# DecaYale/RNNPose

Measured on AMD Instinct MI355X. Metric: pose-refine iters/sec (640x480, B=8, 3x8 recurrent), higher is better.
Workload: dtype f32 (convolutions and volume build: fp16x3-split MFMA, fp32-class accuracy; LM: f64)

## Files before the change

rnnpose_amd/csrc/lm.hip:

```cpp
#include "geometry.cuh"

namespace {

using rp::Intr;
using rp::Pose;

constexpr int NACC = 27;
constexpr int PSTRIDE = 32;
constexpr int LM_THREADS = 256;
#ifndef RP_LM_BATCH
#define RP_LM_BATCH 8
#endif
#ifndef RP_LM_PPB
#define RP_LM_PPB 4096
#endif
constexpr int LM_BATCH = RP_LM_BATCH;
constexpr int LM_PIX_PER_BLOCK = RP_LM_PPB;
constexpr int LM_MAX_BLOCKS = 256;

__host__ __device__ inline int lm_blocks_per_image(long long P) {
  long long n = (P + LM_PIX_PER_BLOCK - 1) / LM_PIX_PER_BLOCK;
  if (n < 1) n = 1;
  if (n > LM_MAX_BLOCKS) n = LM_MAX_BLOCKS;
  return static_cast<int>(n);
}

__device__ __forceinline__ double shfl_down_f64(double v, int d) {
  int lo = __double2loint(v), hi = __double2hiint(v);
  lo = __shfl_down(lo, d);
  hi = __shfl_down(hi, d);
  return __hiloint2double(hi, lo);
}

struct LmTail {
  int* tickets;
  double* Hm;
  double* bv;
  const float* G_in;
  float* G_out;
  float* xi;
  int* info;
  double ep, lm, max_update;
};
__device__ void lm_finalize_block_one(const double* __restrict__ partials, int nblk, int b, double* __restrict__ Hm, double* __restrict__ bv);
__device__ __forceinline__ void lm_solve_one(const double* Hm, const double* bv, const float* G, int b, double ep, double lm, double max_update,
                             float* G_new, float* xi_out, int* info);

__device__ __forceinline__ void lm_accumulate(double (&acc)[NACC], float wgt, float dep, float tx, float ty, int x, int y, int target_mode,
                                          float eps, const Intr& k, const Pose& g) {
  const float Z = dep + eps;
  if (target_mode != 0) {
    tx += static_cast<float>(x);
    ty += static_cast<float>(y);
  }
  const rp::Reproj r = rp::reproject(Z, static_cast<float>(x), static_cast<float>(y), k, g);
  const bool valid = (r.Z0 > rp::kMinDepthValid) && (r.Z1 > rp::kMinDepthValid);
  const double vw = valid ? static_cast<double>(wgt) : 0.0;
  const bool tiny = r.Zc <= rp::kMinDepthProj + 0.01f;
  const float zi1 = tiny ? 0.f : 1.0f / r.Zc;
  const float zi2 = tiny ? 0.f : 1.0f / (r.Zc * r.Zc);
  const double a = static_cast<double>(k.fx * zi1);
  const double c = static_cast<double>(-k.fx * r.X1 * zi2);
  const double d = static_cast<double>(k.fy * zi1);
  const double e = static_cast<double>(-k.fy * r.Y1 * zi2);
  const double X1 = r.X1, Y1 = r.Y1, Z1 = r.Z1;
  double J0[6], J1[6];
  J0[0] = a;   J0[1] = 0.0; J0[2] = c; J0[3] = c * Y1;            J0[4] = a * Z1 + c * (-X1); J0[5] = a * (-Y1);
  J1[0] = 0.0; J1[1] = d;   J1[2] = e; J1[3] = d * (-Z1) + e * Y1; J1[4] = e * (-X1);          J1[5] = d * X1;
  const double r0 = static_cast<double>(tx) - static_cast<double>(r.u);
  const double r1 = static_cast<double>(ty) - static_cast<double>(r.v);
  int idx = 0;
#pragma unroll
  for (int i = 0; i < 6; ++i) {
    const double wi0 = vw * J0[i], wi1 = vw * J1[i];
#pragma unroll
    for (int jj = i; jj < 6; ++jj) {
      acc[idx] += wi0 * J0[jj] + wi1 * J1[jj];
      ++idx;
    }
    acc[21 + i] += wi0 * r0 + wi1 * r1;
  }
}

template <bool FUSED>
__device__ __forceinline__ void lm_reduce_tail(double (&acc)[NACC], double* __restrict__ partials, const LmTail& tail, int b, int nblk, int bx) {
  __shared__ double red[LM_THREADS / 64][NACC];
  __shared__ int is_last;
  const int lane = threadIdx.x & 63, wave = threadIdx.x >> 6;
  {
    double v[32];
#pragma unroll
    for (int i = 0; i < 32; ++i) v[i] = i < NACC ? acc[i] : 0.0;
#pragma unroll
    for (int o = 32, n = 32; o >= 2; o >>= 1, n >>= 1) {
      const bool hi = (lane & o) != 0;
#pragma unroll
      for (int i = 0; i < n / 2; ++i) {
        const double send = hi ? v[i] : v[i + n / 2];
        const double keep = hi ? v[i + n / 2] : v[i];
        v[i] = keep + rp::shfl_xor_f64(send, o);
      }
    }
    const double tot = v[0] + rp::shfl_xor_f64(v[0], 1);
    const int slot = ((lane >> 5) & 1) * 16 + ((lane >> 4) & 1) * 8 + ((lane >> 3) & 1) * 4 + ((lane >> 2) & 1) * 2 + ((lane >> 1) & 1);
    if (!(lane & 1) && slot < NACC) red[wave][slot] = tot;
  }
  __syncthreads();
  if (threadIdx.x < NACC) {
    double v = red[0][threadIdx.x];
#pragma unroll
    for (int wv = 1; wv < LM_THREADS / 64; ++wv) v += red[wv][threadIdx.x];
    partials[(static_cast<long long>(b) * nblk + bx) * PSTRIDE + threadIdx.x] = v;
  }
  if constexpr (FUSED) {
    asm volatile("s_waitcnt vmcnt(0)" ::: "memory");
    __syncthreads();
    if (threadIdx.x == 0) {
      __builtin_amdgcn_fence(__ATOMIC_RELEASE, "agent");
      asm volatile("s_waitcnt vmcnt(0)" ::: "memory");
      const int t = __hip_atomic_fetch_add(&tail.tickets[b], 1, __ATOMIC_RELAXED, __HIP_MEMORY_SCOPE_AGENT);
      is_last = (t == nblk - 1) ? 1 : 0;
      if (is_last) {
        __hip_atomic_store(&tail.tickets[b], 0, __ATOMIC_RELAXED, __HIP_MEMORY_SCOPE_AGENT);
        __builtin_amdgcn_fence(__ATOMIC_ACQUIRE, "agent");
      }
    }
    __syncthreads();
    if (!is_last) return;
    lm_finalize_block_one(partials, nblk, b, tail.Hm, tail.bv);
    __syncthreads();
    if (threadIdx.x == 0) lm_solve_one(tail.Hm, tail.bv, tail.G_in, b, tail.ep, tail.lm, tail.max_update, tail.G_out, tail.xi, tail.info);
  }
}

template <bool FUSED>
__global__ __launch_bounds__(LM_THREADS) void lm_normal_eq_kernel(const float* __restrict__ target, int target_mode,
                                                                  const float* __restrict__ weight,
                                                                  const float* __restrict__ depth, float eps,
                                                                  const float* __restrict__ K,
                                                                  const float* __restrict__ G, int H, int W,
                                                                  double* __restrict__ partials, const LmTail tail) {
  const int b = blockIdx.y;
  const int nblk = gridDim.x;
  const long long P = static_cast<long long>(H) * W;
  const Intr k = rp::load_intr(K, b);
  const Pose g = rp::load_pose(G, b);
  double acc[NACC];
#pragma unroll
  for (int i = 0; i < NACC; ++i) acc[i] = 0.0;

  const long long stride = static_cast<long long>(nblk) * LM_THREADS;
  for (long long t0 = static_cast<long long>(blockIdx.x) * LM_THREADS + threadIdx.x; t0 < P; t0 += LM_BATCH * stride) {
    float wgt_[LM_BATCH], dep_[LM_BATCH], tx_[LM_BATCH], ty_[LM_BATCH];
#pragma unroll
    for (int j = 0; j < LM_BATCH; ++j) {
      const long long tj = t0 + j * stride;
      const long long t = tj < P ? tj : P - 1;
      wgt_[j] = weight[b * P + t];
      dep_[j] = depth[b * P + t];
      if (target_mode == 0) {
        const float2 tt = *reinterpret_cast<const float2*>(target + (b * P + t) * 2);
        tx_[j] = tt.x;
        ty_[j] = tt.y;
      } else {
        tx_[j] = target[(static_cast<long long>(b) * 2 + 0) * P + t];
        ty_[j] = target[(static_cast<long long>(b) * 2 + 1) * P + t];
      }
    }
    __builtin_amdgcn_sched_barrier(0);
#pragma unroll
    for (int j = 0; j < LM_BATCH; ++j) {
      const long long t = t0 + j * stride;
      if (t >= P) break;
      const unsigned tu = static_cast<unsigned>(t);
      const int y = static_cast<int>(tu / static_cast<unsigned>(W)), x = static_cast<int>(tu - static_cast<unsigned>(y) * static_cast<unsigned>(W));
      const float wgt = wgt_[j];
      const bool skippable = wgt == 0.f && __builtin_isfinite(tx_[j]) && __builtin_isfinite(ty_[j]) && __builtin_isfinite(dep_[j]);
      if (__builtin_amdgcn_ballot_w64(!skippable) == 0ull) continue;
      lm_accumulate(acc, wgt, dep_[j], tx_[j], ty_[j], x, y, target_mode, eps, k, g);
    }
  }
  lm_reduce_tail<FUSED>(acc, partials, tail, b, nblk, static_cast<int>(blockIdx.x));
}

__device__ void lm_finalize_block_one(const double* __restrict__ partials, int nblk, int b, double* __restrict__ Hm,
                                      double* __restrict__ bv) {
  __shared__ double grp[8][PSTRIDE];
  __shared__ double s[NACC];
  const int k = threadIdx.x & 31, g = threadIdx.x >> 5;
  double v = 0.0;
  for (int i = g; i < nblk; i += 8) v += partials[(static_cast<long long>(b) * nblk + i) * PSTRIDE + k];
  grp[g][k] = v;
  __syncthreads();
  if (threadIdx.x < NACC) {
    double t = 0.0;
    for (int q = 0; q < 8; ++q) t += grp[q][threadIdx.x];
    s[threadIdx.x] = t;
  }
  __syncthreads();
  if (threadIdx.x < 36) {
    const int i = threadIdx.x / 6, j = threadIdx.x % 6;
    const int r = i < j ? i : j, c = i < j ? j : i;
    const int idx = r * 6 - r * (r - 1) / 2 + (c - r);
    Hm[b * 36 + threadIdx.x] = s[idx];
  } else if (threadIdx.x < 42) {
    bv[b * 6 + (threadIdx.x - 36)] = s[21 + (threadIdx.x - 36)];
  }
}

__global__ __launch_bounds__(256) void lm_finalize_kernel(const double* __restrict__ partials, int nblk,
                                                          double* __restrict__ Hm, double* __restrict__ bv) {
  lm_finalize_block_one(partials, nblk, blockIdx.x, Hm, bv);
}

__device__ void se3_exp_dev(const float* xi, float* Gout ) {
  const float v0 = xi[0], v1 = xi[1], v2 = xi[2];
  const float w0 = xi[3], w1 = xi[4], w2 = xi[5];
  const float th2 = w0 * w0 + w1 * w1 + w2 * w2;
  const float th = sqrtf(th2);
  const float th4 = th2 * th2;
  const float wx[9] = {0.f, -w2, w1, w2, 0.f, -w0, -w1, w0, 0.f};
  float wx2[9];
  for (int i = 0; i < 3; ++i)
    for (int j = 0; j < 3; ++j) wx2[i * 3 + j] = wx[i * 3 + 0] * wx[0 * 3 + j] + wx[i * 3 + 1] * wx[1 * 3 + j] + wx[i * 3 + 2] * wx[2 * 3 + j];
  float A, Bc, Cc;
  float Bv;
  const float eps = 1e-12f;
  if (th < rp::kMinTheta) {
    A = 1.0f - (1.0f / 6.0f) * th2 + (1.0f / 120.0f) * th4;
    Bc = 0.5f - (1.0f / 12.0f) * th2 + (1.0f / 720.0f) * th4;
    Bv = 0.5f - (1.0f / 24.0f) * th2 + (1.0f / 720.0f) * th4;
    Cc = (1.0f / 6.0f) - (1.0f / 120.0f) * th2 + (1.0f / 5040.0f) * th4;
  } else {
    A = sinf(th) / (th + eps);
    Bc = (1.0f - cosf(th)) / (th2 + eps);
    Bv = Bc;
    Cc = (th - sinf(th)) / (th2 * th + eps);
  }
  float Rm[9], Vm[9];
  for (int i = 0; i < 9; ++i) {
    const float I = (i == 0 || i == 4 || i == 8) ? 1.f : 0.f;
    Rm[i] = I + A * wx[i] + Bc * wx2[i];
    Vm[i] = I + Bv * wx[i] + Cc * wx2[i];
  }
  for (int i = 0; i < 3; ++i) {
    Gout[i * 4 + 0] = Rm[i * 3 + 0];
    Gout[i * 4 + 1] = Rm[i * 3 + 1];
    Gout[i * 4 + 2] = Rm[i * 3 + 2];
    Gout[i * 4 + 3] = Vm[i * 3 + 0] * v0 + Vm[i * 3 + 1] * v1 + Vm[i * 3 + 2] * v2;
  }
  Gout[12] = 0.f; Gout[13] = 0.f; Gout[14] = 0.f; Gout[15] = 1.f;
}

__device__ void mat4_mul(const float* A, const float* Bm, float* C) {
  for (int i = 0; i < 4; ++i)
    for (int j = 0; j < 4; ++j) {
      float s = 0.f;
      for (int k = 0; k < 4; ++k) s += A[i * 4 + k] * Bm[k * 4 + j];
      C[i * 4 + j] = s;
    }
}

__device__ __forceinline__ void lm_solve_one(const double* Hm, const double* bv, const float* G, int b, double ep, double lm,
                                             double max_update, float* G_new , float* xi_out, int* info) {
  double L[21], xv[6];
#define LT(i_, j_) L[(i_) * ((i_) + 1) / 2 + (j_)]
#pragma unroll
  for (int i = 0; i < 6; ++i) {
#pragma unroll
    for (int j = 0; j <= i; ++j) LT(i, j) = Hm[b * 36 + i * 6 + j];
    xv[i] = bv[b * 6 + i];
  }
#pragma unroll
  for (int i = 0; i < 6; ++i) LT(i, i) = LT(i, i) + ep + lm * LT(i, i);
  int bad = 0;
  const double nan = __longlong_as_double(0x7ff8000000000000LL);
#pragma unroll
  for (int j = 0; j < 6; ++j) {
    double s = LT(j, j);
#pragma unroll
    for (int k = 0; k < j; ++k) s -= LT(j, k) * LT(j, k);
    if (!(s > 0.0)) {
      if (!bad) bad = j + 1;
      LT(j, j) = nan;
    } else {
      LT(j, j) = sqrt(s);
    }
#pragma unroll
    for (int i = j + 1; i < 6; ++i) {
      double t = LT(i, j);
#pragma unroll
      for (int k = 0; k < j; ++k) t -= LT(i, k) * LT(j, k);
      LT(i, j) = t / LT(j, j);
    }
  }
#pragma unroll
  for (int i = 0; i < 6; ++i) {
    double t = xv[i];
#pragma unroll
    for (int k = 0; k < i; ++k) t -= LT(i, k) * xv[k];
    xv[i] = t / LT(i, i);
  }
#pragma unroll
  for (int i = 5; i >= 0; --i) {
    double t = xv[i];
#pragma unroll
    for (int k = i + 1; k < 6; ++k) t -= LT(k, i) * xv[k];
    xv[i] = t / LT(i, i);
  }
#undef LT
  float xi[6];
  for (int i = 0; i < 6; ++i) {
    double v = xv[i];
    if (v != v) v = 0.0;
    v = v < -max_update ? -max_update : (v > max_update ? max_update : v);
    xi[i] = static_cast<float>(v);
    xi_out[b * 6 + i] = xi[i];
  }
  if (info) info[b] = bad;
  float dG[16], Gin[16], Gout[16];
  se3_exp_dev(xi, dG);
  for (int i = 0; i < 16; ++i) Gin[i] = G[b * 16 + i];
  mat4_mul(dG, Gin, Gout);
  for (int i = 0; i < 16; ++i) G_new[b * 16 + i] = Gout[i];
}

__global__ __launch_bounds__(64) void lm_solve_update_kernel(const double* __restrict__ Hm, const double* __restrict__ bv,
                                                             const float* G, int B, double ep, double lm,
                                                             double max_update, float* G_new ,
                                                             float* __restrict__ xi_out, int* __restrict__ info) {
  const int b = blockIdx.x * blockDim.x + threadIdx.x;
  if (b < B) lm_solve_one(Hm, bv, G, b, ep, lm, max_update, G_new, xi_out, info);
}

__global__ void se3_exp_kernel(const float* __restrict__ xi, int B, float* __restrict__ out) {
  const int b = blockIdx.x * blockDim.x + threadIdx.x;
  if (b >= B) return;
  float x[6], Gm[16];
  for (int i = 0; i < 6; ++i) x[i] = xi[b * 6 + i];
  se3_exp_dev(x, Gm);
  for (int i = 0; i < 16; ++i) out[b * 16 + i] = Gm[i];
}

__global__ void se3_compose_kernel(const float* __restrict__ A, const float* __restrict__ Bm, int B, float* __restrict__ out) {
  const int b = blockIdx.x * blockDim.x + threadIdx.x;
  if (b >= B) return;
  float a[16], c[16], o[16];
  for (int i = 0; i < 16; ++i) {
    a[i] = A[b * 16 + i];
    c[i] = Bm[b * 16 + i];
  }
  mat4_mul(a, c, o);
  for (int i = 0; i < 16; ++i) out[b * 16 + i] = o[i];
}

__global__ void se3_inverse_kernel(const float* __restrict__ A, int B, float* __restrict__ out) {
  const int b = blockIdx.x * blockDim.x + threadIdx.x;
  if (b >= B) return;
  float a[16], o[16];
  for (int i = 0; i < 16; ++i) a[i] = A[b * 16 + i];
  for (int i = 0; i < 3; ++i) {
    for (int j = 0; j < 3; ++j) o[i * 4 + j] = a[j * 4 + i];
    float s = 0.f;
    for (int k = 0; k < 3; ++k) s += a[k * 4 + i] * a[k * 4 + 3];
    o[i * 4 + 3] = -s;
  }
  o[12] = 0.f; o[13] = 0.f; o[14] = 0.f; o[15] = 1.f;
  for (int i = 0; i < 16; ++i) out[b * 16 + i] = o[i];
}

__global__ void se3_outer_update_kernel(const float* __restrict__ Tij, const float* __restrict__ Ti, int B, int literal, float* __restrict__ Ti_out,
                                        float* __restrict__ Tij_out) {
  const int b = blockIdx.x * blockDim.x + threadIdx.x;
  if (b >= B) return;
  float a[16], c[16], t[16], inv[16], o[16];
  for (int i = 0; i < 16; ++i) {
    a[i] = Tij[b * 16 + i];
    c[i] = Ti[b * 16 + i];
  }
  mat4_mul(a, c, t);
  for (int i = 0; i < 16; ++i) Ti_out[b * 16 + i] = t[i];
  if (literal) {
    for (int i = 0; i < 3; ++i) {
      for (int j = 0; j < 3; ++j) inv[i * 4 + j] = t[j * 4 + i];
      float s = 0.f;
      for (int k = 0; k < 3; ++k) s += t[k * 4 + i] * t[k * 4 + 3];
      inv[i * 4 + 3] = -s;
    }
    inv[12] = 0.f; inv[13] = 0.f; inv[14] = 0.f; inv[15] = 1.f;
    mat4_mul(t, inv, o);
  } else {
    for (int i = 0; i < 16; ++i) o[i] = (i % 5 == 0) ? 1.f : 0.f;
  }
  for (int i = 0; i < 16; ++i) Tij_out[b * 16 + i] = o[i];
}

inline double* lm_partials(void* workspace, int B) { return static_cast<double*>(workspace) + B; }

int launch_normal_eq_partials(const float* target, int target_mode, const float* weight, const float* depth, float eps,
                              const float* K, const float* G, int B, int H, int W, void* workspace, hipStream_t st) {
  const long long P = static_cast<long long>(H) * W;
  const int nblk = lm_blocks_per_image(P);
  hipLaunchKernelGGL(lm_normal_eq_kernel<false>, dim3(nblk, B), dim3(LM_THREADS), 0, st, target, target_mode, weight, depth, eps,
                     K, G, H, W, lm_partials(workspace, B), LmTail{});
  return nblk;
}

void launch_lm_step_fused(const float* target, int target_mode, const float* weight, const float* depth, float eps, const float* K,
                          const float* G_in, float* G_out, int B, int H, int W, double ep, double lm, double max_update,
                          void* workspace, double* Hm, double* bv, float* xi, int* info, hipStream_t st) {
  const long long P = static_cast<long long>(H) * W;
  const int nblk = lm_blocks_per_image(P);
  LmTail tail{};
  tail.tickets = static_cast<int*>(workspace);
  tail.Hm = Hm; tail.bv = bv; tail.G_in = G_in; tail.G_out = G_out; tail.xi = xi; tail.info = info;
  tail.ep = ep; tail.lm = lm; tail.max_update = max_update;
  hipLaunchKernelGGL(lm_normal_eq_kernel<true>, dim3(nblk, B), dim3(LM_THREADS), 0, st, target, target_mode, weight, depth, eps,
                     K, G_in, H, W, lm_partials(workspace, B), tail);
}

int launch_normal_eq(const float* target, int target_mode, const float* weight, const float* depth, float eps,
                     const float* K, const float* G, int B, int H, int W, void* workspace, double* Hm, double* bv,
                     hipStream_t st) {
  const int nblk = launch_normal_eq_partials(target, target_mode, weight, depth, eps, K, G, B, H, W, workspace, st);
  hipLaunchKernelGGL(lm_finalize_kernel, dim3(B), dim3(256), 0, st, lm_partials(workspace, B), nblk, Hm, bv);
  return 0;
}

}

extern "C" {

size_t rnnpose_lm_workspace_bytes(int B, int H, int W) {
  if (B <= 0 || H <= 0 || W <= 0) return 0;
  return static_cast<size_t>(B) * lm_blocks_per_image(static_cast<long long>(H) * W) * PSTRIDE * sizeof(double) +
         static_cast<size_t>(B) * sizeof(double);
}

static bool g_lm_fused = true;
int rnnpose_lm_fused_tail(int enable) {
  g_lm_fused = enable != 0;
  return 0;
}

int rnnpose_lm_normal_eq_f64(const float* target, int target_mode, const float* weight, const float* depth,
                             float depth_eps, const float* K, const float* G, int B, int H, int W, void* workspace,
                             size_t workspace_bytes, double* Hm, double* bv, rnnpose_stream_t stream) {
  const char* fn = "rnnpose_lm_normal_eq_f64";
  RP_REQUIRE(target && weight && depth && K && G && workspace && Hm && bv, fn, "null pointer");
  RP_REQUIRE(target_mode == 0 || target_mode == 1, fn, "target_mode must be 0 or 1");
  RP_REQUIRE(B > 0 && B < 65536 && H > 0 && W > 0 && static_cast<long long>(H) * W < (1LL << 31), fn, "bad size");
  RP_REQUIRE(workspace_bytes >= rnnpose_lm_workspace_bytes(B, H, W), fn, "workspace too small");
  launch_normal_eq(target, target_mode, weight, depth, depth_eps, K, G, B, H, W, workspace, Hm, bv, rp::as_stream(stream));
  return rp::check_launch(fn);
}

int rnnpose_lm_solve_update_f32(const double* Hm, const double* bv, const float* G, int B, double ep_lambda,
                                double lm_lambda, double max_update, float* G_new, float* xi, int* info,
                                rnnpose_stream_t stream) {
  const char* fn = "rnnpose_lm_solve_update_f32";
  RP_REQUIRE(Hm && bv && G && G_new && xi, fn, "null pointer");
  RP_REQUIRE(B > 0, fn, "bad size");
  hipLaunchKernelGGL(lm_solve_update_kernel, dim3(rp::cdiv(B, 64)), dim3(64), 0, rp::as_stream(stream), Hm, bv, G, B,
                     ep_lambda, lm_lambda, max_update, G_new, xi, info);
  return rp::check_launch(fn);
}

static int lm_step_impl(const char* fn, const float* target, int target_mode, const float* weight, const float* depth,
                        float depth_eps, const float* K, const float* G_in, float* G_out, int B, int H, int W, int num_iters,
                        double ep_lambda, double lm_lambda, double max_update, void* workspace, size_t workspace_bytes,
                        double* Hm, double* bv, float* xi, int* info, rnnpose_stream_t stream) {
  RP_REQUIRE(target && weight && depth && K && G_in && G_out && workspace && Hm && bv && xi, fn, "null pointer");
  RP_REQUIRE(target_mode == 0 || target_mode == 1, fn, "target_mode must be 0 or 1");
  RP_REQUIRE(B > 0 && B < 65536 && H > 0 && W > 0 && static_cast<long long>(H) * W < (1LL << 31) && num_iters >= 0, fn, "bad size");
  RP_REQUIRE(workspace_bytes >= rnnpose_lm_workspace_bytes(B, H, W), fn, "workspace too small");
  hipStream_t st = rp::as_stream(stream);
  for (int it = 0; it < num_iters; ++it) {
    const float* g = it == 0 ? G_in : G_out;
    if (g_lm_fused && info) {
      launch_lm_step_fused(target, target_mode, weight, depth, depth_eps, K, g, G_out, B, H, W, ep_lambda, lm_lambda, max_update,
                           workspace, Hm, bv, xi, info, st);
      continue;
    }
    launch_normal_eq(target, target_mode, weight, depth, depth_eps, K, g, B, H, W, workspace, Hm, bv, st);
    hipLaunchKernelGGL(lm_solve_update_kernel, dim3(rp::cdiv(B, 64)), dim3(64), 0, st, Hm, bv, g, B, ep_lambda,
                       lm_lambda, max_update, G_out, xi, info);
  }
  return rp::check_launch(fn);
}

int rnnpose_lm_step_f32(const float* target, int target_mode, const float* weight, const float* depth, float depth_eps,
                        const float* K, float* G, int B, int H, int W, int num_iters, double ep_lambda, double lm_lambda,
                        double max_update, void* workspace, size_t workspace_bytes, double* Hm, double* bv, float* xi,
                        int* info, rnnpose_stream_t stream) {
  return lm_step_impl("rnnpose_lm_step_f32", target, target_mode, weight, depth, depth_eps, K, G, G, B, H, W, num_iters,
                      ep_lambda, lm_lambda, max_update, workspace, workspace_bytes, Hm, bv, xi, info, stream);
}

int rnnpose_lm_step_io_f32(const float* target, int target_mode, const float* weight, const float* depth, float depth_eps,
                           const float* K, const float* G_in, float* G_out, int B, int H, int W, int num_iters,
                           double ep_lambda, double lm_lambda, double max_update, void* workspace, size_t workspace_bytes,
                           double* Hm, double* bv, float* xi, int* info, rnnpose_stream_t stream) {
  RP_REQUIRE(num_iters >= 1, "rnnpose_lm_step_io_f32", "needs at least one iteration (G_out would stay unwritten)");
  return lm_step_impl("rnnpose_lm_step_io_f32", target, target_mode, weight, depth, depth_eps, K, G_in, G_out, B, H, W,
                      num_iters, ep_lambda, lm_lambda, max_update, workspace, workspace_bytes, Hm, bv, xi, info, stream);
}

int rnnpose_se3_exp_f32(const float* xi, int B, float* out, rnnpose_stream_t stream) {
  const char* fn = "rnnpose_se3_exp_f32";
  RP_REQUIRE(xi && out && B > 0, fn, "bad argument");
  hipLaunchKernelGGL(se3_exp_kernel, dim3(rp::cdiv(B, 64)), dim3(64), 0, rp::as_stream(stream), xi, B, out);
  return rp::check_launch(fn);
}

int rnnpose_se3_compose_f32(const float* A, const float* Bm, int B, float* out, rnnpose_stream_t stream) {
  const char* fn = "rnnpose_se3_compose_f32";
  RP_REQUIRE(A && Bm && out && B > 0, fn, "bad argument");
  hipLaunchKernelGGL(se3_compose_kernel, dim3(rp::cdiv(B, 64)), dim3(64), 0, rp::as_stream(stream), A, Bm, B, out);
  return rp::check_launch(fn);
}

int rnnpose_se3_outer_update_f32(const float* Tij, const float* Ti, int B, int literal, float* Ti_out, float* Tij_out, rnnpose_stream_t stream) {
  const char* fn = "rnnpose_se3_outer_update_f32";
  RP_REQUIRE(Tij && Ti && Ti_out && Tij_out && B > 0, fn, "null pointer / empty batch");
  hipLaunchKernelGGL(se3_outer_update_kernel, dim3(rp::cdiv(B, 64)), dim3(64), 0, rp::as_stream(stream), Tij, Ti, B, literal, Ti_out, Tij_out);
  return rp::check_launch(fn);
}

int rnnpose_se3_inverse_f32(const float* A, int B, float* out, rnnpose_stream_t stream) {
  const char* fn = "rnnpose_se3_inverse_f32";
  RP_REQUIRE(A && out && B > 0, fn, "bad argument");
  hipLaunchKernelGGL(se3_inverse_kernel, dim3(rp::cdiv(B, 64)), dim3(64), 0, rp::as_stream(stream), A, B, out);
  return rp::check_launch(fn);
}

}
```

Measured before the change: 745.9.

## Add LM system kernel with fewer larger blocks and parallel partial-record reduction

Adds a new default LM normal-equation kernel that uses 512-thread blocks, caps the grid at 64 blocks per image, and batches 10 pixels per thread. The Jacobian accumulation now uses explicit FMAs and skips the structurally zero terms. The last-arriving block sums the per-block partials in parallel across thread groups and solves from shared memory. The aim is to cut the serial finalize and reduction cost and the tail latency of the fused LM step. The trade-off is fewer blocks in flight, which may leave less parallelism to hide memory latency. It also adds ablation macros for experiments.

```diff
diff --git a/rnnpose_amd/csrc/lm.hip b/rnnpose_amd/csrc/lm.hip
--- a/rnnpose_amd/csrc/lm.hip
+++ b/rnnpose_amd/csrc/lm.hip
@@ -13,6 +13,12 @@
 #endif
 #ifndef RP_LM_PPB
 #define RP_LM_PPB 4096
+#endif
+#ifndef LM_V2
+#define LM_V2 1
+#endif
+#ifndef RP_LM_ABL
+#define RP_LM_ABL 0
 #endif
 constexpr int LM_BATCH = RP_LM_BATCH;
 constexpr int LM_PIX_PER_BLOCK = RP_LM_PPB;
@@ -43,8 +49,8 @@
   double ep, lm, max_update;
 };
 __device__ void lm_finalize_block_one(const double* __restrict__ partials, int nblk, int b, double* __restrict__ Hm, double* __restrict__ bv);
-__device__ __forceinline__ void lm_solve_one(const double* Hm, const double* bv, const float* G, int b, double ep, double lm, double max_update,
-                             float* G_new, float* xi_out, int* info);
+__device__ __forceinline__ void lm_solve_one(const double* H, const double* bh, const float* Gb, int b, double ep, double lm, double max_update,
+                                             float* G_new, float* xi_out, int* info);
 
 __device__ __forceinline__ void lm_accumulate(double (&acc)[NACC], float wgt, float dep, float tx, float ty, int x, int y, int target_mode,
                                           float eps, const Intr& k, const Pose& g) {
@@ -82,29 +88,48 @@
   }
 }
 
+__device__ __forceinline__ void lm_wave_reduce(double (&acc)[NACC], double* red_row) {
+  const int lane = threadIdx.x & 63;
+  double v[32];
+#pragma unroll
+  for (int i = 0; i < 32; ++i) v[i] = i < NACC ? acc[i] : 0.0;
+#pragma unroll
+  for (int o = 32, n = 32; o >= 2; o >>= 1, n >>= 1) {
+    const bool hi = (lane & o) != 0;
+#pragma unroll
+    for (int i = 0; i < n / 2; ++i) {
+      const double send = hi ? v[i] : v[i + n / 2];
+      const double keep = hi ? v[i + n / 2] : v[i];
+      v[i] = keep + rp::shfl_xor_f64(send, o);
+    }
+  }
+  const double tot = v[0] + rp::shfl_xor_f64(v[0], 1);
+  const int slot = ((lane >> 5) & 1) * 16 + ((lane >> 4) & 1) * 8 + ((lane >> 3) & 1) * 4 + ((lane >> 2) & 1) * 2 + ((lane >> 1) & 1);
+  if (!(lane & 1) && slot < NACC) red_row[slot] = tot;
+}
+
+__device__ __forceinline__ bool lm_last_arrival(int* tickets, int b, int nblk) {
+  __shared__ int is_last;
+  asm volatile("s_waitcnt vmcnt(0)" ::: "memory");
+  __syncthreads();
+  if (threadIdx.x == 0) {
+    __builtin_amdgcn_fence(__ATOMIC_RELEASE, "agent");
+    asm volatile("s_waitcnt vmcnt(0)" ::: "memory");
+    const int t = __hip_atomic_fetch_add(&tickets[b], 1, __ATOMIC_RELAXED, __HIP_MEMORY_SCOPE_AGENT);
+    is_last = (t == nblk - 1) ? 1 : 0;
+    if (is_last) {
+      __hip_atomic_store(&tickets[b], 0, __ATOMIC_RELAXED, __HIP_MEMORY_SCOPE_AGENT);
+      __builtin_amdgcn_fence(__ATOMIC_ACQUIRE, "agent");
+    }
+  }
+  __syncthreads();
+  return is_last != 0;
+}
+
 template <bool FUSED>
 __device__ __forceinline__ void lm_reduce_tail(double (&acc)[NACC], double* __restrict__ partials, const LmTail& tail, int b, int nblk, int bx) {
   __shared__ double red[LM_THREADS / 64][NACC];
-  __shared__ int is_last;
-  const int lane = threadIdx.x & 63, wave = threadIdx.x >> 6;
-  {
-    double v[32];
-#pragma unroll
-    for (int i = 0; i < 32; ++i) v[i] = i < NACC ? acc[i] : 0.0;
-#pragma unroll
-    for (int o = 32, n = 32; o >= 2; o >>= 1, n >>= 1) {
-      const bool hi = (lane & o) != 0;
-#pragma unroll
-      for (int i = 0; i < n / 2; ++i) {
-        const double send = hi ? v[i] : v[i + n / 2];
-        const double keep = hi ? v[i + n / 2] : v[i];
-        v[i] = keep + rp::shfl_xor_f64(send, o);
-      }
-    }
-    const double tot = v[0] + rp::shfl_xor_f64(v[0], 1);
-    const int slot = ((lane >> 5) & 1) * 16 + ((lane >> 4) & 1) * 8 + ((lane >> 3) & 1) * 4 + ((lane >> 2) & 1) * 2 + ((lane >> 1) & 1);
-    if (!(lane & 1) && slot < NACC) red[wave][slot] = tot;
-  }
+  lm_wave_reduce(acc, red[threadIdx.x >> 6]);
   __syncthreads();
   if (threadIdx.x < NACC) {
     double v = red[0][threadIdx.x];
@@ -112,24 +137,12 @@
     for (int wv = 1; wv < LM_THREADS / 64; ++wv) v += red[wv][threadIdx.x];
     partials[(static_cast<long long>(b) * nblk + bx) * PSTRIDE + threadIdx.x] = v;
   }
-  if constexpr (FUSED) {
-    asm volatile("s_waitcnt vmcnt(0)" ::: "memory");
-    __syncthreads();
-    if (threadIdx.x == 0) {
-      __builtin_amdgcn_fence(__ATOMIC_RELEASE, "agent");
-      asm volatile("s_waitcnt vmcnt(0)" ::: "memory");
-      const int t = __hip_atomic_fetch_add(&tail.tickets[b], 1, __ATOMIC_RELAXED, __HIP_MEMORY_SCOPE_AGENT);
-      is_last = (t == nblk - 1) ? 1 : 0;
-      if (is_last) {
-        __hip_atomic_store(&tail.tickets[b], 0, __ATOMIC_RELAXED, __HIP_MEMORY_SCOPE_AGENT);
-        __builtin_amdgcn_fence(__ATOMIC_ACQUIRE, "agent");
-      }
-    }
-    __syncthreads();
-    if (!is_last) return;
+  if constexpr (FUSED && RP_LM_ABL != 3) {
+    if (!lm_last_arrival(tail.tickets, b, nblk)) return;
     lm_finalize_block_one(partials, nblk, b, tail.Hm, tail.bv);
     __syncthreads();
-    if (threadIdx.x == 0) lm_solve_one(tail.Hm, tail.bv, tail.G_in, b, tail.ep, tail.lm, tail.max_update, tail.G_out, tail.xi, tail.info);
+    if (threadIdx.x == 0 && RP_LM_ABL != 2)
+      lm_solve_one(tail.Hm + b * 36, tail.bv + b * 6, tail.G_in + b * 16, b, tail.ep, tail.lm, tail.max_update, tail.G_out, tail.xi, tail.info);
   }
 }
 
@@ -177,7 +190,8 @@
       const float wgt = wgt_[j];
       const bool skippable = wgt == 0.f && __builtin_isfinite(tx_[j]) && __builtin_isfinite(ty_[j]) && __builtin_isfinite(dep_[j]);
       if (__builtin_amdgcn_ballot_w64(!skippable) == 0ull) continue;
-      lm_accumulate(acc, wgt, dep_[j], tx_[j], ty_[j], x, y, target_mode, eps, k, g);
+      if (RP_LM_ABL == 1) acc[0] += static_cast<double>(wgt + dep_[j] + tx_[j] + ty_[j] + static_cast<float>(x + y));
+      else lm_accumulate(acc, wgt, dep_[j], tx_[j], ty_[j], x, y, target_mode, eps, k, g);
     }
   }
   lm_reduce_tail<FUSED>(acc, partials, tail, b, nblk, static_cast<int>(blockIdx.x));
@@ -211,6 +225,189 @@
 __global__ __launch_bounds__(256) void lm_finalize_kernel(const double* __restrict__ partials, int nblk,
                                                           double* __restrict__ Hm, double* __restrict__ bv) {
   lm_finalize_block_one(partials, nblk, blockIdx.x, Hm, bv);
+}
+
+#ifndef RP_LM2_THREADS
+#define RP_LM2_THREADS 512
+#endif
+#ifndef RP_LM2_BLOCKS
+#define RP_LM2_BLOCKS 64
+#endif
+#ifndef RP_LM2_BATCH
+#define RP_LM2_BATCH 10
+#endif
+constexpr int LM2_THREADS = RP_LM2_THREADS;
+constexpr int LM2_BLOCKS = RP_LM2_BLOCKS;
+constexpr int LM2_BATCH = RP_LM2_BATCH;
+constexpr int LM2_MIN_PIX = 1024;
+constexpr int LM2_GROUPS = LM2_THREADS / 32;
+constexpr int LM2_REC_PER_GROUP = (LM2_BLOCKS + LM2_GROUPS - 1) / LM2_GROUPS;
+static_assert(LM2_THREADS % 64 == 0 && LM2_THREADS <= 1024 && LM2_BLOCKS <= LM_MAX_BLOCKS, "LM_V2 geometry");
+
+__host__ __device__ inline int lm2_blocks_per_image(long long P) {
+  long long n = (P + LM2_MIN_PIX - 1) / LM2_MIN_PIX;
+  if (n < 1) n = 1;
+  if (n > LM2_BLOCKS) n = LM2_BLOCKS;
+  return static_cast<int>(n);
+}
+
+__device__ __forceinline__ void lm2_sum_records(const double* __restrict__ partials, int nblk, int b, double* s) {
+  __shared__ double grp[LM2_GROUPS][PSTRIDE];
+  const int k = threadIdx.x & 31, q = threadIdx.x >> 5;
+  const double* rec = partials + static_cast<long long>(b) * nblk * PSTRIDE + k;
+  double x[LM2_REC_PER_GROUP];
+#pragma unroll
+  for (int j = 0; j < LM2_REC_PER_GROUP; ++j) {
+    const int i = q + j * LM2_GROUPS;
+    x[j] = rec[(i < nblk ? i : nblk - 1) * PSTRIDE];
+  }
+  double v = 0.0;
+#pragma unroll
+  for (int j = 0; j < LM2_REC_PER_GROUP; ++j)
+    if (q + j * LM2_GROUPS < nblk) v += x[j];
+  grp[q][k] = v;
+  __syncthreads();
+  if (threadIdx.x < NACC) {
+    double t = 0.0;
+    for (int g = 0; g < LM2_GROUPS; ++g) t += grp[g][threadIdx.x];
+    s[threadIdx.x] = t;
+  }
+  __syncthreads();
+}
+
+__device__ __forceinline__ void lm2_expand(const double* s, double* H36, double* b6) {
+  if (threadIdx.x < 36) {
+    const int i = threadIdx.x / 6, j = threadIdx.x % 6;
+    const int r = i < j ? i : j, c = i < j ? j : i;
+    H36[threadIdx.x] = s[r * 6 - r * (r - 1) / 2 + (c - r)];
+  } else if (threadIdx.x < 42) {
+    b6[threadIdx.x - 36] = s[21 + (threadIdx.x - 36)];
+  }
+}
+
+__device__ __forceinline__ void lm2_accumulate(double (&acc)[NACC], float wgt, float dep, float tx, float ty, int x, int y, int target_mode,
+                                               float eps, const Intr& k, const Pose& g) {
+  const float Z = dep + eps;
+  if (target_mode != 0) {
+    tx += static_cast<float>(x);
+    ty += static_cast<float>(y);
+  }
+  const rp::Reproj r = rp::reproject(Z, static_cast<float>(x), static_cast<float>(y), k, g);
+  const bool valid = (r.Z0 > rp::kMinDepthValid) && (r.Z1 > rp::kMinDepthValid);
+  const double vw = valid ? static_cast<double>(wgt) : 0.0;
+  const bool tiny = r.Zc <= rp::kMinDepthProj + 0.01f;
+  const float zi1 = tiny ? 0.f : 1.0f / r.Zc;
+  const float zi2 = tiny ? 0.f : 1.0f / (r.Zc * r.Zc);
+  const double a = static_cast<double>(k.fx * zi1);
+  const double c = static_cast<double>(-k.fx * r.X1 * zi2);
+  const double d = static_cast<double>(k.fy * zi1);
+  const double e = static_cast<double>(-k.fy * r.Y1 * zi2);
+  const double X1 = r.X1, Y1 = r.Y1, Z1 = r.Z1;
+  const double P[6] = {a, 0.0, c, c * Y1, a * Z1 + c * (-X1), a * (-Y1)};
+  const double Q[6] = {0.0, d, e, d * (-Z1) + e * Y1, e * (-X1), d * X1};
+  const double r0 = static_cast<double>(tx) - static_cast<double>(r.u);
+  const double r1 = static_cast<double>(ty) - static_cast<double>(r.v);
+  double wp[6], wq[6];
+#pragma unroll
+  for (int i = 0; i < 6; ++i) {
+    wp[i] = vw * P[i];
+    wq[i] = vw * Q[i];
+  }
+  int idx = 0;
+#pragma unroll
+  for (int i = 0; i < 6; ++i) {
+#pragma unroll
+    for (int jj = i; jj < 6; ++jj) {
+      if (i == 0 && jj == 1) {
+        acc[idx] = fma(wp[0], P[1], acc[idx]);
+      } else {
+        if (i != 1 && jj != 1) acc[idx] = fma(wp[i], P[jj], acc[idx]);
+        if (i != 0 && jj != 0) acc[idx] = fma(wq[i], Q[jj], acc[idx]);
+      }
+      ++idx;
+    }
+    if (i != 1) acc[21 + i] = fma(wp[i], r0, acc[21 + i]);
+    if (i != 0) acc[21 + i] = fma(wq[i], r1, acc[21 + i]);
+  }
+}
+
+template <bool FUSED>
+__global__ __launch_bounds__(LM2_THREADS) void lm_system_kernel(const float* __restrict__ target, int target_mode,
+                                                                const float* __restrict__ weight, const float* __restrict__ depth,
+                                                                float eps, const float* __restrict__ K, const float* __restrict__ G,
+                                                                int H, int W, double* __restrict__ partials, const LmTail tail) {
+  __shared__ double red[LM2_THREADS / 64][NACC];
+  __shared__ double sys[NACC], sH[36], sb[6];
+  __shared__ float sG[16];
+  const int b = blockIdx.y;
+  const int nblk = gridDim.x;
+  const long long P = static_cast<long long>(H) * W;
+  const Intr k = rp::load_intr(K, b);
+  const Pose g = rp::load_pose(G, b);
+  if (FUSED && threadIdx.x < 16) sG[threadIdx.x] = G[b * 16 + threadIdx.x];
+  double acc[NACC];
+#pragma unroll
+  for (int i = 0; i < NACC; ++i) acc[i] = 0.0;
+
+  const float* wb = weight + b * P;
+  const float* db = depth + b * P;
+  const long long stride = static_cast<long long>(nblk) * LM2_THREADS;
+  for (long long t0 = static_cast<long long>(blockIdx.x) * LM2_THREADS + threadIdx.x; t0 < P; t0 += LM2_BATCH * stride) {
+    float wgt_[LM2_BATCH], dep_[LM2_BATCH], tx_[LM2_BATCH], ty_[LM2_BATCH];
+#pragma unroll
+    for (int j = 0; j < LM2_BATCH; ++j) {
+      const long long tj = t0 + j * stride;
+      const long long t = tj < P ? tj : P - 1;
+      wgt_[j] = wb[t];
+      dep_[j] = db[t];
+      if (target_mode == 0) {
+        const float2 tt = *reinterpret_cast<const float2*>(target + (b * P + t) * 2);
+        tx_[j] = tt.x;
+        ty_[j] = tt.y;
+      } else {
+        tx_[j] = target[(static_cast<long long>(b) * 2 + 0) * P + t];
+        ty_[j] = target[(static_cast<long long>(b) * 2 + 1) * P + t];
+      }
+    }
+    __builtin_amdgcn_sched_barrier(0);
+#pragma unroll
+    for (int j = 0; j < LM2_BATCH; ++j) {
+      const long long t = t0 + j * stride;
+      if (t >= P) break;
+      const unsigned tu = static_cast<unsigned>(t);
+      const int y = static_cast<int>(tu / static_cast<unsigned>(W)), x = static_cast<int>(tu - static_cast<unsigned>(y) * static_cast<unsigned>(W));
+      const float wgt = wgt_[j];
+      const bool skippable = wgt == 0.f && __builtin_isfinite(tx_[j]) && __builtin_isfinite(ty_[j]) && __builtin_isfinite(dep_[j]);
+      if (__builtin_amdgcn_ballot_w64(!skippable) == 0ull) continue;
+      if (RP_LM_ABL == 1) acc[0] += static_cast<double>(wgt + dep_[j] + tx_[j] + ty_[j] + static_cast<float>(x + y));
+      else lm2_accumulate(acc, wgt, dep_[j], tx_[j], ty_[j], x, y, target_mode, eps, k, g);
+    }
+  }
+
+  lm_wave_reduce(acc, red[threadIdx.x >> 6]);
+  __syncthreads();
+  if (threadIdx.x < NACC) {
+    double v = red[0][threadIdx.x];
+#pragma unroll
+    for (int wv = 1; wv < LM2_THREADS / 64; ++wv) v += red[wv][threadIdx.x];
+    partials[(static_cast<long long>(b) * nblk + blockIdx.x) * PSTRIDE + threadIdx.x] = v;
+  }
+  if constexpr (FUSED && RP_LM_ABL != 3) {
+    if (!lm_last_arrival(tail.tickets, b, nblk)) return;
+    lm2_sum_records(partials, nblk, b, sys);
+    lm2_expand(sys, tail.Hm + b * 36, tail.bv + b * 6);
+    if (RP_LM_ABL == 2) return;
+    lm2_expand(sys, sH, sb);
+    __syncthreads();
+    if (threadIdx.x == 0) lm_solve_one(sH, sb, sG, b, tail.ep, tail.lm, tail.max_update, tail.G_out, tail.xi, tail.info);
+  }
+}
+
+__global__ __launch_bounds__(LM2_THREADS) void lm_system_finalize_kernel(const double* __restrict__ partials, int nblk,
+                                                                         double* __restrict__ Hm, double* __restrict__ bv) {
+  __shared__ double sys[NACC];
+  lm2_sum_records(partials, nblk, blockIdx.x, sys);
+  lm2_expand(sys, Hm + blockIdx.x * 36, bv + blockIdx.x * 6);
 }
 
 __device__ void se3_exp_dev(const float* xi, float* Gout ) {
@@ -261,15 +458,15 @@
     }
 }
 
-__device__ __forceinline__ void lm_solve_one(const double* Hm, const double* bv, const float* G, int b, double ep, double lm,
+__device__ __forceinline__ void lm_solve_one(const double* H, const double* bh, const float* Gb, int b, double ep, double lm,
                                              double max_update, float* G_new , float* xi_out, int* info) {
   double L[21], xv[6];
 #define LT(i_, j_) L[(i_) * ((i_) + 1) / 2 + (j_)]
 #pragma unroll
   for (int i = 0; i < 6; ++i) {
 #pragma unroll
-    for (int j = 0; j <= i; ++j) LT(i, j) = Hm[b * 36 + i * 6 + j];
-    xv[i] = bv[b * 6 + i];
+    for (int j = 0; j <= i; ++j) LT(i, j) = H[i * 6 + j];
+    xv[i] = bh[i];
   }
 #pragma unroll
   for (int i = 0; i < 6; ++i) LT(i, i) = LT(i, i) + ep + lm * LT(i, i);
@@ -320,7 +517,7 @@
   if (info) info[b] = bad;
   float dG[16], Gin[16], Gout[16];
   se3_exp_dev(xi, dG);
-  for (int i = 0; i < 16; ++i) Gin[i] = G[b * 16 + i];
+  for (int i = 0; i < 16; ++i) Gin[i] = Gb[i];
   mat4_mul(dG, Gin, Gout);
   for (int i = 0; i < 16; ++i) G_new[b * 16 + i] = Gout[i];
 }
@@ -330,7 +527,7 @@
                                                              double max_update, float* G_new ,
                                                              float* __restrict__ xi_out, int* __restrict__ info) {
   const int b = blockIdx.x * blockDim.x + threadIdx.x;
-  if (b < B) lm_solve_one(Hm, bv, G, b, ep, lm, max_update, G_new, xi_out, info);
+  if (b < B) lm_solve_one(Hm + b * 36, bv + b * 6, G + b * 16, b, ep, lm, max_update, G_new, xi_out, info);
 }
 
 __global__ void se3_exp_kernel(const float* __restrict__ xi, int B, float* __restrict__ out) {
@@ -397,33 +594,40 @@
 
 inline double* lm_partials(void* workspace, int B) { return static_cast<double*>(workspace) + B; }
 
-int launch_normal_eq_partials(const float* target, int target_mode, const float* weight, const float* depth, float eps,
-                              const float* K, const float* G, int B, int H, int W, void* workspace, hipStream_t st) {
+inline int lm_records_per_image(long long P) { return LM_V2 ? lm2_blocks_per_image(P) : lm_blocks_per_image(P); }
+
+template <bool FUSED>
+void launch_system(const float* target, int target_mode, const float* weight, const float* depth, float eps, const float* K,
+                   const float* G, int B, int H, int W, void* workspace, const LmTail& tail, hipStream_t st) {
   const long long P = static_cast<long long>(H) * W;
-  const int nblk = lm_blocks_per_image(P);
-  hipLaunchKernelGGL(lm_normal_eq_kernel<false>, dim3(nblk, B), dim3(LM_THREADS), 0, st, target, target_mode, weight, depth, eps,
-                     K, G, H, W, lm_partials(workspace, B), LmTail{});
-  return nblk;
+  const int nblk = lm_records_per_image(P);
+  if (LM_V2)
+    hipLaunchKernelGGL(lm_system_kernel<FUSED>, dim3(nblk, B), dim3(LM2_THREADS), 0, st, target, target_mode, weight, depth, eps,
+                       K, G, H, W, lm_partials(workspace, B), tail);
+  else
+    hipLaunchKernelGGL(lm_normal_eq_kernel<FUSED>, dim3(nblk, B), dim3(LM_THREADS), 0, st, target, target_mode, weight, depth, eps,
+                       K, G, H, W, lm_partials(workspace, B), tail);
 }
 
 void launch_lm_step_fused(const float* target, int target_mode, const float* weight, const float* depth, float eps, const float* K,
                           const float* G_in, float* G_out, int B, int H, int W, double ep, double lm, double max_update,
                           void* workspace, double* Hm, double* bv, float* xi, int* info, hipStream_t st) {
-  const long long P = static_cast<long long>(H) * W;
-  const int nblk = lm_blocks_per_image(P);
   LmTail tail{};
   tail.tickets = static_cast<int*>(workspace);
   tail.Hm = Hm; tail.bv = bv; tail.G_in = G_in; tail.G_out = G_out; tail.xi = xi; tail.info = info;
   tail.ep = ep; tail.lm = lm; tail.max_update = max_update;
-  hipLaunchKernelGGL(lm_normal_eq_kernel<true>, dim3(nblk, B), dim3(LM_THREADS), 0, st, target, target_mode, weight, depth, eps,
-                     K, G_in, H, W, lm_partials(workspace, B), tail);
+  launch_system<true>(target, target_mode, weight, depth, eps, K, G_in, B, H, W, workspace, tail, st);
 }
 
 int launch_normal_eq(const float* target, int target_mode, const float* weight, const float* depth, float eps,
                      const float* K, const float* G, int B, int H, int W, void* workspace, double* Hm, double* bv,
                      hipStream_t st) {
-  const int nblk = launch_normal_eq_partials(target, target_mode, weight, depth, eps, K, G, B, H, W, workspace, st);
-  hipLaunchKernelGGL(lm_finalize_kernel, dim3(B), dim3(256), 0, st, lm_partials(workspace, B), nblk, Hm, bv);
+  launch_system<false>(target, target_mode, weight, depth, eps, K, G, B, H, W, workspace, LmTail{}, st);
+  const int nblk = lm_records_per_image(static_cast<long long>(H) * W);
+  if (LM_V2)
+    hipLaunchKernelGGL(lm_system_finalize_kernel, dim3(B), dim3(LM2_THREADS), 0, st, lm_partials(workspace, B), nblk, Hm, bv);
+  else
+    hipLaunchKernelGGL(lm_finalize_kernel, dim3(B), dim3(256), 0, st, lm_partials(workspace, B), nblk, Hm, bv);
   return 0;
 }
 
@@ -433,7 +637,9 @@
 
 size_t rnnpose_lm_workspace_bytes(int B, int H, int W) {
   if (B <= 0 || H <= 0 || W <= 0) return 0;
-  return static_cast<size_t>(B) * lm_blocks_per_image(static_cast<long long>(H) * W) * PSTRIDE * sizeof(double) +
+  const long long P = static_cast<long long>(H) * W;
+  const int nrec = lm_blocks_per_image(P) > lm2_blocks_per_image(P) ? lm_blocks_per_image(P) : lm2_blocks_per_image(P);
+  return static_cast<size_t>(B) * nrec * PSTRIDE * sizeof(double) +
          static_cast<size_t>(B) * sizeof(double);
 }
 
```

Measured after the change: 750.6, median of 6. About the same (+0.6%).
